# argumentcomputer/lurk-beta

Measured on NVIDIA B200. Metric: Lurk iterations proved/sec (fib rc=100, Nova IVC), higher is better.
Workload: dtype u32x8 (254-bit Montgomery integers)

## Files before the change

lurk-beta_b200/csrc/field.cuh:

```cuda
#pragma once
#include <cstdint>
#include <cstring>

#if defined(__CUDACC__)
#define LURK_HD __host__ __device__ __forceinline__
#define LURK_D __device__ __forceinline__
#else
#define LURK_HD inline
#define LURK_D inline
#endif

#include "field_consts.cuh"

namespace lurk {

namespace cc {
#if defined(__CUDA_ARCH__)
LURK_D uint32_t add_cc(uint32_t a, uint32_t b) { uint32_t r; asm volatile("add.cc.u32 %0, %1, %2;" : "=r"(r) : "r"(a), "r"(b)); return r; }
LURK_D uint32_t addc_cc(uint32_t a, uint32_t b) { uint32_t r; asm volatile("addc.cc.u32 %0, %1, %2;" : "=r"(r) : "r"(a), "r"(b)); return r; }
LURK_D uint32_t addc(uint32_t a, uint32_t b) { uint32_t r; asm volatile("addc.u32 %0, %1, %2;" : "=r"(r) : "r"(a), "r"(b)); return r; }
LURK_D uint32_t sub_cc(uint32_t a, uint32_t b) { uint32_t r; asm volatile("sub.cc.u32 %0, %1, %2;" : "=r"(r) : "r"(a), "r"(b)); return r; }
LURK_D uint32_t subc_cc(uint32_t a, uint32_t b) { uint32_t r; asm volatile("subc.cc.u32 %0, %1, %2;" : "=r"(r) : "r"(a), "r"(b)); return r; }
LURK_D uint32_t subc(uint32_t a, uint32_t b) { uint32_t r; asm volatile("subc.u32 %0, %1, %2;" : "=r"(r) : "r"(a), "r"(b)); return r; }
LURK_D uint32_t mul_lo(uint32_t a, uint32_t b) { uint32_t r; asm volatile("mul.lo.u32 %0, %1, %2;" : "=r"(r) : "r"(a), "r"(b)); return r; }
LURK_D uint32_t mul_hi(uint32_t a, uint32_t b) { uint32_t r; asm volatile("mul.hi.u32 %0, %1, %2;" : "=r"(r) : "r"(a), "r"(b)); return r; }
LURK_D uint32_t mad_lo_cc(uint32_t a, uint32_t b, uint32_t c) { uint32_t r; asm volatile("mad.lo.cc.u32 %0, %1, %2, %3;" : "=r"(r) : "r"(a), "r"(b), "r"(c)); return r; }
LURK_D uint32_t madc_lo_cc(uint32_t a, uint32_t b, uint32_t c) { uint32_t r; asm volatile("madc.lo.cc.u32 %0, %1, %2, %3;" : "=r"(r) : "r"(a), "r"(b), "r"(c)); return r; }
LURK_D uint32_t mad_hi_cc(uint32_t a, uint32_t b, uint32_t c) { uint32_t r; asm volatile("mad.hi.cc.u32 %0, %1, %2, %3;" : "=r"(r) : "r"(a), "r"(b), "r"(c)); return r; }
LURK_D uint32_t madc_hi_cc(uint32_t a, uint32_t b, uint32_t c) { uint32_t r; asm volatile("madc.hi.cc.u32 %0, %1, %2, %3;" : "=r"(r) : "r"(a), "r"(b), "r"(c)); return r; }
LURK_D uint32_t madc_hi(uint32_t a, uint32_t b, uint32_t c) { uint32_t r; asm volatile("madc.hi.u32 %0, %1, %2, %3;" : "=r"(r) : "r"(a), "r"(b), "r"(c)); return r; }
#else
inline uint32_t &cf() { static thread_local uint32_t f = 0; return f; }
inline uint32_t add_cc(uint32_t a, uint32_t b) { uint64_t s = (uint64_t)a + b; cf() = (uint32_t)(s >> 32); return (uint32_t)s; }
inline uint32_t addc_cc(uint32_t a, uint32_t b) { uint64_t s = (uint64_t)a + b + cf(); cf() = (uint32_t)(s >> 32); return (uint32_t)s; }
inline uint32_t addc(uint32_t a, uint32_t b) { return a + b + cf(); }
inline uint32_t sub_cc(uint32_t a, uint32_t b) { uint64_t d = (uint64_t)a - b; cf() = (uint32_t)(d >> 63); return (uint32_t)d; }
inline uint32_t subc_cc(uint32_t a, uint32_t b) { uint64_t d = (uint64_t)a - b - cf(); cf() = (uint32_t)(d >> 63); return (uint32_t)d; }
inline uint32_t subc(uint32_t a, uint32_t b) { return a - b - cf(); }
inline uint32_t mul_lo(uint32_t a, uint32_t b) { return a * b; }
inline uint32_t mul_hi(uint32_t a, uint32_t b) { return (uint32_t)(((uint64_t)a * b) >> 32); }
inline uint32_t mad_lo_cc(uint32_t a, uint32_t b, uint32_t c) { uint64_t s = (uint64_t)(a * b) + c; cf() = (uint32_t)(s >> 32); return (uint32_t)s; }
inline uint32_t madc_lo_cc(uint32_t a, uint32_t b, uint32_t c) { uint64_t s = (uint64_t)(a * b) + c + cf(); cf() = (uint32_t)(s >> 32); return (uint32_t)s; }
inline uint32_t mad_hi_cc(uint32_t a, uint32_t b, uint32_t c) { uint64_t s = (((uint64_t)a * b) >> 32) + c; cf() = (uint32_t)(s >> 32); return (uint32_t)s; }
inline uint32_t madc_hi_cc(uint32_t a, uint32_t b, uint32_t c) { uint64_t s = (((uint64_t)a * b) >> 32) + c + cf(); cf() = (uint32_t)(s >> 32); return (uint32_t)s; }
inline uint32_t madc_hi(uint32_t a, uint32_t b, uint32_t c) { return (uint32_t)(((uint64_t)a * b) >> 32) + c + cf(); }
#endif
}

template <class P>
struct alignas(16) Fe {
    uint32_t v[8];
    using Params = P;

    LURK_HD static Fe zero() { Fe r; for (int i = 0; i < 8; i++) r.v[i] = 0; return r; }
    LURK_HD static Fe one() { Fe r; for (int i = 0; i < 8; i++) r.v[i] = P::ONE(i); return r; }
    LURK_HD static Fe rr() { Fe r; for (int i = 0; i < 8; i++) r.v[i] = P::RR(i); return r; }
    LURK_HD static Fe modulus_raw() { Fe r; for (int i = 0; i < 8; i++) r.v[i] = P::MOD(i); return r; }

    LURK_HD bool is_zero() const { uint32_t o = 0; for (int i = 0; i < 8; i++) o |= v[i]; return o == 0; }
    LURK_HD bool operator==(const Fe &b) const { uint32_t o = 0; for (int i = 0; i < 8; i++) o |= v[i] ^ b.v[i]; return o == 0; }
    LURK_HD bool operator!=(const Fe &b) const { return !(*this == b); }

    LURK_HD void final_sub() {
        uint32_t t[8];
        t[0] = cc::sub_cc(v[0], P::MOD(0));
#pragma unroll
        for (int i = 1; i < 8; i++) t[i] = cc::subc_cc(v[i], P::MOD(i));
        uint32_t borrow = cc::subc(0, 0);
#pragma unroll
        for (int i = 0; i < 8; i++) v[i] = borrow ? v[i] : t[i];
    }
    LURK_HD bool is_reduced() const {
        uint32_t t = cc::sub_cc(v[0], P::MOD(0));
#pragma unroll
        for (int i = 1; i < 8; i++) t = cc::subc_cc(v[i], P::MOD(i));
        (void)t;
        return cc::subc(0, 0) != 0;
    }

    LURK_HD friend Fe operator+(const Fe &a, const Fe &b) {
        Fe r;
        r.v[0] = cc::add_cc(a.v[0], b.v[0]);
#pragma unroll
        for (int i = 1; i < 7; i++) r.v[i] = cc::addc_cc(a.v[i], b.v[i]);
        r.v[7] = cc::addc(a.v[7], b.v[7]);
        r.final_sub();
        return r;
    }
    LURK_HD friend Fe operator-(const Fe &a, const Fe &b) {
        Fe r;
        r.v[0] = cc::sub_cc(a.v[0], b.v[0]);
#pragma unroll
        for (int i = 1; i < 8; i++) r.v[i] = cc::subc_cc(a.v[i], b.v[i]);
        uint32_t borrow = cc::subc(0, 0);
        r.v[0] = cc::add_cc(r.v[0], P::MOD(0) & borrow);
#pragma unroll
        for (int i = 1; i < 7; i++) r.v[i] = cc::addc_cc(r.v[i], P::MOD(i) & borrow);
        r.v[7] = cc::addc(r.v[7], P::MOD(7) & borrow);
        return r;
    }
    LURK_HD Fe neg() const { return zero() - *this; }
    LURK_HD Fe dbl() const { return *this + *this; }

    LURK_HD static void mul_n(uint32_t *acc, const uint32_t *a, uint32_t bi) {
#pragma unroll
        for (int j = 0; j < 8; j += 2) { acc[j] = cc::mul_lo(a[j], bi); acc[j + 1] = cc::mul_hi(a[j], bi); }
    }
    LURK_HD static void cmad_n(uint32_t *acc, const uint32_t *a, uint32_t bi) {
        acc[0] = cc::mad_lo_cc(a[0], bi, acc[0]);
        acc[1] = cc::madc_hi_cc(a[0], bi, acc[1]);
#pragma unroll
        for (int j = 2; j < 8; j += 2) { acc[j] = cc::madc_lo_cc(a[j], bi, acc[j]); acc[j + 1] = cc::madc_hi_cc(a[j], bi, acc[j + 1]); }
    }
    template <int OFF>
    LURK_HD static void cmad_mod(uint32_t *acc, uint32_t mi) {
        acc[0] = cc::mad_lo_cc(P::MOD(OFF), mi, acc[0]);
        acc[1] = cc::madc_hi_cc(P::MOD(OFF), mi, acc[1]);
#pragma unroll
        for (int j = 2; j < 8; j += 2) { acc[j] = cc::madc_lo_cc(P::MOD(OFF + j), mi, acc[j]); acc[j + 1] = cc::madc_hi_cc(P::MOD(OFF + j), mi, acc[j + 1]); }
    }
    LURK_HD static void madc_n_rshift(uint32_t *odd, const uint32_t *a, uint32_t bi) {
#pragma unroll
        for (int j = 0; j < 6; j += 2) { odd[j] = cc::madc_lo_cc(a[j], bi, odd[j + 2]); odd[j + 1] = cc::madc_hi_cc(a[j], bi, odd[j + 3]); }
        odd[6] = cc::madc_lo_cc(a[6], bi, 0);
        odd[7] = cc::madc_hi(a[6], bi, 0);
    }
    template <bool FIRST>
    LURK_HD static void mad_row_redc(uint32_t *even, uint32_t *odd, const uint32_t *a, uint32_t bi) {
        if (FIRST) {
            mul_n(odd, a + 1, bi);
            mul_n(even, a, bi);
        } else {
            even[0] = cc::add_cc(even[0], odd[1]);
            madc_n_rshift(odd, a + 1, bi);
            cmad_n(even, a, bi);
            odd[7] = cc::addc(odd[7], 0);
        }
        uint32_t mi = even[0] * P::M0;
        cmad_mod<1>(odd, mi);
        cmad_mod<0>(even, mi);
        odd[7] = cc::addc(odd[7], 0);
    }

    LURK_HD friend Fe operator*(const Fe &a, const Fe &b) {
#if !defined(__CUDA_ARCH__) && !defined(LURK_HOST_EMULATE_CC)
        return host_mul(a, b);
#else
        uint32_t even[8], odd[8];
        mad_row_redc<true>(even, odd, a.v, b.v[0]);
        mad_row_redc<false>(odd, even, a.v, b.v[1]);
#pragma unroll
        for (int i = 2; i < 8; i += 2) {
            mad_row_redc<false>(even, odd, a.v, b.v[i]);
            mad_row_redc<false>(odd, even, a.v, b.v[i + 1]);
        }
        Fe r;
        r.v[0] = cc::add_cc(even[0], odd[1]);
#pragma unroll
        for (int i = 1; i < 7; i++) r.v[i] = cc::addc_cc(even[i], odd[i + 1]);
        r.v[7] = cc::addc(even[7], 0);
        r.final_sub();
        return r;
#endif
    }
#if !defined(__CUDA_ARCH__)
    static Fe host_mul(const Fe &a, const Fe &b) {
        typedef unsigned __int128 u128;
        uint64_t A[4], B[4], M[4], t[6] = {0, 0, 0, 0, 0, 0};
        for (int i = 0; i < 4; i++) {
            A[i] = (uint64_t)a.v[2 * i] | ((uint64_t)a.v[2 * i + 1] << 32);
            B[i] = (uint64_t)b.v[2 * i] | ((uint64_t)b.v[2 * i + 1] << 32);
            M[i] = (uint64_t)P::MOD(2 * i) | ((uint64_t)P::MOD(2 * i + 1) << 32);
        }
        uint64_t inv = 1;
        for (int i = 0; i < 6; i++) inv *= 2 - M[0] * inv;
        inv = 0 - inv;
        for (int i = 0; i < 4; i++) {
            uint64_t c = 0;
            for (int j = 0; j < 4; j++) { u128 s = (u128)A[j] * B[i] + t[j] + c; t[j] = (uint64_t)s; c = (uint64_t)(s >> 64); }
            u128 s = (u128)t[4] + c; t[4] = (uint64_t)s; t[5] = (uint64_t)(s >> 64);
            uint64_t m = t[0] * inv;
            s = (u128)m * M[0] + t[0]; c = (uint64_t)(s >> 64);
            for (int j = 1; j < 4; j++) { s = (u128)m * M[j] + t[j] + c; t[j - 1] = (uint64_t)s; c = (uint64_t)(s >> 64); }
            s = (u128)t[4] + c; t[3] = (uint64_t)s; t[4] = t[5] + (uint64_t)(s >> 64);
        }
        bool ge = t[4] != 0;
        if (!ge) {
            ge = true;
            for (int i = 3; i >= 0; i--) { if (t[i] > M[i]) break; if (t[i] < M[i]) { ge = false; break; } }
        }
        if (ge) { uint64_t br = 0; for (int i = 0; i < 4; i++) { u128 d = (u128)t[i] - M[i] - br; t[i] = (uint64_t)d; br = (uint64_t)(d >> 64) & 1; } }
        Fe r;
        for (int i = 0; i < 4; i++) { r.v[2 * i] = (uint32_t)t[i]; r.v[2 * i + 1] = (uint32_t)(t[i] >> 32); }
        return r;
    }
#endif
    LURK_HD Fe sqr() const { return *this * *this; }
    LURK_HD Fe pow5() const { Fe x2 = sqr(); Fe x4 = x2.sqr(); return x4 * *this; }

    LURK_HD Fe &operator+=(const Fe &b) { *this = *this + b; return *this; }
    LURK_HD Fe &operator-=(const Fe &b) { *this = *this - b; return *this; }
    LURK_HD Fe &operator*=(const Fe &b) { *this = *this * b; return *this; }

    LURK_HD static Fe from_canonical(const Fe &raw) { return raw * rr(); }
    LURK_HD Fe to_canonical() const {
        Fe o = zero();
        o.v[0] = 1;
        return *this * o;
    }
    LURK_HD static Fe from_u64(uint64_t x) {
        Fe r = zero();
        r.v[0] = (uint32_t)x;
        r.v[1] = (uint32_t)(x >> 32);
        return from_canonical(r);
    }

    LURK_HD Fe pow_raw(const uint32_t e[8]) const {
        Fe acc = one(), base = *this;
        for (int i = 0; i < 256; i++) {
            if ((e[i >> 5] >> (i & 31)) & 1) acc = acc * base;
            base = base.sqr();
        }
        return acc;
    }
    LURK_HD Fe inv_vartime() const {
        if (is_zero()) return zero();
        uint32_t u[8], w[8];
        Fe x1 = zero(), x2 = zero();
        x1.v[0] = 1;
#pragma unroll
        for (int i = 0; i < 8; i++) { u[i] = v[i]; w[i] = P::MOD(i); }
        auto is_one = [](const uint32_t *a) { uint32_t o = a[0] ^ 1u; for (int i = 1; i < 8; i++) o |= a[i]; return o == 0; };
        auto shr1 = [](uint32_t *a) { for (int i = 0; i < 7; i++) a[i] = (a[i] >> 1) | (a[i + 1] << 31); a[7] >>= 1; };
        auto halve = [&](Fe &x) {
            if (x.v[0] & 1u) {
                x.v[0] = cc::add_cc(x.v[0], P::MOD(0));
                for (int i = 1; i < 7; i++) x.v[i] = cc::addc_cc(x.v[i], P::MOD(i));
                x.v[7] = cc::addc(x.v[7], P::MOD(7));
            }
            shr1(x.v);
        };
        auto sub_raw = [](uint32_t *a, const uint32_t *b) {
            a[0] = cc::sub_cc(a[0], b[0]);
            for (int i = 1; i < 8; i++) a[i] = cc::subc_cc(a[i], b[i]);
            return cc::subc(0, 0);
        };
        auto geq = [](const uint32_t *a, const uint32_t *b) {
            for (int i = 7; i >= 0; i--) { if (a[i] > b[i]) return true; if (a[i] < b[i]) return false; }
            return true;
        };
        while (!is_one(u) && !is_one(w)) {
            while (!(u[0] & 1u)) { shr1(u); halve(x1); }
            while (!(w[0] & 1u)) { shr1(w); halve(x2); }
            if (geq(u, w)) { sub_raw(u, w); x1 = x1 - x2; }
            else { sub_raw(w, u); x2 = x2 - x1; }
        }
        const Fe r3 = rr() * rr();
        return (is_one(u) ? x1 : x2) * r3;
    }
    LURK_HD Fe inv() const {
        uint32_t e[8];
        e[0] = cc::sub_cc(P::MOD(0), 2);
#pragma unroll
        for (int i = 1; i < 8; i++) e[i] = cc::subc_cc(P::MOD(i), 0);
        return pow_raw(e);
    }
};

template <class P, int ROUNDS>
LURK_HD Fe<P> redc17(uint32_t *t) {
    uint32_t r[9];
#pragma unroll
    for (int k = 0; k < 9; k++) r[k] = 0;
#pragma unroll
    for (int i = 0; i < 8; i++) {
        uint32_t mi = t[i] * P::M0;
        Fe<P>::template cmad_mod<0>(t + i, mi);
        r[i] = cc::addc(r[i], 0);
        Fe<P>::template cmad_mod<1>(t + i + 1, mi);
        r[i + 1] = cc::addc(r[i + 1], 0);
    }
    t[8] = cc::add_cc(t[8], r[0]);
#pragma unroll
    for (int k = 1; k < 8; k++) t[8 + k] = cc::addc_cc(t[8 + k], r[k]);
    t[16] = cc::addc(t[16], r[8]);
#pragma unroll
    for (int round = 0; round < ROUNDS; round++) {
        uint32_t d[9];
        d[0] = cc::sub_cc(t[8], P::MOD(0));
#pragma unroll
        for (int k = 1; k < 8; k++) d[k] = cc::subc_cc(t[8 + k], P::MOD(k));
        d[8] = cc::subc_cc(t[16], 0);
        uint32_t borrow = cc::subc(0, 0);
#pragma unroll
        for (int k = 0; k < 9; k++) t[8 + k] = borrow ? t[8 + k] : d[k];
    }
    Fe<P> out;
#pragma unroll
    for (int k = 0; k < 8; k++) out.v[k] = t[8 + k];
    return out;
}

template <class P>
struct WideAcc {
    uint32_t e[17];
    uint32_t o[16];
    uint32_t ce[5];
    uint32_t co[4];

    LURK_HD void clear() {
#pragma unroll
        for (int i = 0; i < 17; i++) e[i] = 0;
#pragma unroll
        for (int i = 0; i < 16; i++) o[i] = 0;
#pragma unroll
        for (int i = 0; i < 5; i++) ce[i] = 0;
#pragma unroll
        for (int i = 0; i < 4; i++) co[i] = 0;
    }

    template <int I>
    LURK_HD void row(const uint32_t *a, uint32_t bi) {
        if (I % 2 == 0) {
            Fe<P>::cmad_n(e + I, a, bi);
            ce[I / 2] = cc::addc(ce[I / 2], 0);
            Fe<P>::cmad_n(o + I, a + 1, bi);
            co[I / 2] = cc::addc(co[I / 2], 0);
        } else {
            Fe<P>::cmad_n(e + I + 1, a + 1, bi);
            ce[(I + 1) / 2] = cc::addc(ce[(I + 1) / 2], 0);
            Fe<P>::cmad_n(o + I - 1, a, bi);
            co[(I - 1) / 2] = cc::addc(co[(I - 1) / 2], 0);
        }
    }
    LURK_HD void mul_acc(const Fe<P> &a, const Fe<P> &b) {
        row<0>(a.v, b.v[0]); row<1>(a.v, b.v[1]); row<2>(a.v, b.v[2]); row<3>(a.v, b.v[3]);
        row<4>(a.v, b.v[4]); row<5>(a.v, b.v[5]); row<6>(a.v, b.v[6]); row<7>(a.v, b.v[7]);
    }

    template <int ROUNDS = 3>
    LURK_HD Fe<P> reduce() {
        e[8] = cc::add_cc(e[8], ce[0]);   e[9] = cc::addc_cc(e[9], 0);
        e[10] = cc::addc_cc(e[10], ce[1]); e[11] = cc::addc_cc(e[11], 0);
        e[12] = cc::addc_cc(e[12], ce[2]); e[13] = cc::addc_cc(e[13], 0);
        e[14] = cc::addc_cc(e[14], ce[3]); e[15] = cc::addc_cc(e[15], 0);
        e[16] = cc::addc(e[16], ce[4]);
        o[8] = cc::add_cc(o[8], co[0]);   o[9] = cc::addc_cc(o[9], 0);
        o[10] = cc::addc_cc(o[10], co[1]); o[11] = cc::addc_cc(o[11], 0);
        o[12] = cc::addc_cc(o[12], co[2]); o[13] = cc::addc_cc(o[13], 0);
        o[14] = cc::addc_cc(o[14], co[3]); o[15] = cc::addc(o[15], 0);
        uint32_t t[17];
        t[0] = e[0];
        t[1] = cc::add_cc(e[1], o[0]);
#pragma unroll
        for (int k = 2; k < 16; k++) t[k] = cc::addc_cc(e[k], o[k - 1]);
        t[16] = cc::addc(e[16], o[15]);
        return redc17<P, ROUNDS>(t);
    }
};

template <class F>
LURK_D F load_fe(const void *p) {
#if defined(__CUDA_ARCH__)
    const uint4 *q = reinterpret_cast<const uint4 *>(p);
    uint4 lo = q[0], hi = q[1];
    F r;
    r.v[0] = lo.x; r.v[1] = lo.y; r.v[2] = lo.z; r.v[3] = lo.w;
    r.v[4] = hi.x; r.v[5] = hi.y; r.v[6] = hi.z; r.v[7] = hi.w;
    return r;
#else
    F r; memcpy(r.v, p, 32); return r;
#endif
}
template <class F>
LURK_D void store_fe(void *p, const F &x) {
#if defined(__CUDA_ARCH__)
    uint4 *q = reinterpret_cast<uint4 *>(p);
    q[0] = make_uint4(x.v[0], x.v[1], x.v[2], x.v[3]);
    q[1] = make_uint4(x.v[4], x.v[5], x.v[6], x.v[7]);
#else
    memcpy(p, x.v, 32);
#endif
}

}
```

Before: 27770.

## Replace binary extended GCD inversion with batched safegcd over 30-bit limbs

Replaces the bit-by-bit binary extended Euclid field inverse with a Bernstein–Yang style divstep algorithm. It works on signed 30-bit limbs, runs 30 divsteps per batch on low words, and then applies a 2x2 transition matrix to the full-width values with Montgomery-style division by 2^30. This cuts the number of multi-limb passes and the data-dependent branching per bit. In exchange it adds limb conversion, normalisation, and 64-bit multiply work per batch, and carries correctness risk in the sign, delta and modular-reduction handling.

```diff
diff --git a/lurk-beta_b200/csrc/field.cuh b/lurk-beta_b200/csrc/field.cuh
--- a/lurk-beta_b200/csrc/field.cuh
+++ b/lurk-beta_b200/csrc/field.cuh
@@ -223,40 +223,119 @@
         }
         return acc;
     }
+    static constexpr uint32_t M30 = 0x3fffffffu;
+    LURK_HD static void to_s30(const uint32_t *w, int32_t *o) {
+#pragma unroll
+        for (int k = 0; k < 9; k++) {
+            const int bit = 30 * k, word = bit >> 5, sh = bit & 31;
+            uint32_t lo = w[word] >> sh;
+            if (sh > 2 && word + 1 < 8) lo |= w[word + 1] << (32 - sh);
+            o[k] = (int32_t)(lo & M30);
+        }
+    }
+    LURK_HD static Fe from_s30(const int32_t *o) {
+        Fe r;
+        uint64_t acc = 0;
+        int bits = 0, wi = 0;
+#pragma unroll
+        for (int k = 0; k < 9; k++) {
+            acc |= (uint64_t)(uint32_t)o[k] << bits;
+            bits += 30;
+            if (bits >= 32 && wi < 8) { r.v[wi++] = (uint32_t)acc; acc >>= 32; bits -= 32; }
+        }
+        return r;
+    }
+    LURK_HD static uint32_t ctz32(uint32_t x) {
+#if defined(__CUDA_ARCH__)
+        return (uint32_t)(__ffs((int)x) - 1);
+#else
+        return (uint32_t)__builtin_ctz(x);
+#endif
+    }
+
     LURK_HD Fe inv_vartime() const {
         if (is_zero()) return zero();
-        uint32_t u[8], w[8];
-        Fe x1 = zero(), x2 = zero();
-        x1.v[0] = 1;
-#pragma unroll
-        for (int i = 0; i < 8; i++) { u[i] = v[i]; w[i] = P::MOD(i); }
-        auto is_one = [](const uint32_t *a) { uint32_t o = a[0] ^ 1u; for (int i = 1; i < 8; i++) o |= a[i]; return o == 0; };
-        auto shr1 = [](uint32_t *a) { for (int i = 0; i < 7; i++) a[i] = (a[i] >> 1) | (a[i + 1] << 31); a[7] >>= 1; };
-        auto halve = [&](Fe &x) {
-            if (x.v[0] & 1u) {
-                x.v[0] = cc::add_cc(x.v[0], P::MOD(0));
-                for (int i = 1; i < 7; i++) x.v[i] = cc::addc_cc(x.v[i], P::MOD(i));
-                x.v[7] = cc::addc(x.v[7], P::MOD(7));
+        int32_t f[9], g[9], d[9], e[9], pm[9];
+        {
+            uint32_t w[8];
+#pragma unroll
+            for (int i = 0; i < 8; i++) w[i] = P::MOD(i);
+            to_s30(w, pm);
+        }
+#pragma unroll
+        for (int k = 0; k < 9; k++) { f[k] = pm[k]; d[k] = 0; e[k] = 0; }
+        to_s30(v, g);
+        e[0] = 1;
+        int delta2 = 1;
+        auto normalise = [&pm](int32_t *a) {
+            const int32_t neg = a[8] >> 31;
+            int32_t c = 0;
+#pragma unroll
+            for (int k = 0; k < 8; k++) { c += a[k] + (pm[k] & neg); a[k] = c & (int32_t)M30; c >>= 30; }
+            a[8] += c + (pm[8] & neg);
+            int32_t t[9];
+            c = 0;
+#pragma unroll
+            for (int k = 0; k < 8; k++) { c += a[k] - pm[k]; t[k] = c & (int32_t)M30; c >>= 30; }
+            t[8] = a[8] - pm[8] + c;
+            const int32_t keep = t[8] >> 31;
+#pragma unroll
+            for (int k = 0; k < 9; k++) a[k] = (a[k] & keep) | (t[k] & ~keep);
+        };
+#pragma unroll 1
+        for (int batch = 0; batch < 20; batch++) {
+            uint32_t fl = (uint32_t)f[0], gl = (uint32_t)g[0];
+            uint32_t u = 1, vv = 0, q = 0, r = 1;
+            int left = 30;
+#pragma unroll 1
+            for (;;) {
+                const uint32_t z = ctz32(gl | (1u << left));
+                gl >>= z; u <<= z; vv <<= z;
+                delta2 += 2 * (int)z;
+                left -= (int)z;
+                if (left == 0) break;
+                if (delta2 > 0) {
+                    delta2 = 2 - delta2;
+                    uint32_t t = fl; fl = gl; gl -= t;
+                    t = u; u = q; q -= t;
+                    t = vv; vv = r; r -= t;
+                } else {
+                    delta2 += 2;
+                    gl += fl; q += u; r += vv;
+                }
+                gl >>= 1; u <<= 1; vv <<= 1;
+                if (--left == 0) break;
             }
-            shr1(x.v);
-        };
-        auto sub_raw = [](uint32_t *a, const uint32_t *b) {
-            a[0] = cc::sub_cc(a[0], b[0]);
-            for (int i = 1; i < 8; i++) a[i] = cc::subc_cc(a[i], b[i]);
-            return cc::subc(0, 0);
-        };
-        auto geq = [](const uint32_t *a, const uint32_t *b) {
-            for (int i = 7; i >= 0; i--) { if (a[i] > b[i]) return true; if (a[i] < b[i]) return false; }
-            return true;
-        };
-        while (!is_one(u) && !is_one(w)) {
-            while (!(u[0] & 1u)) { shr1(u); halve(x1); }
-            while (!(w[0] & 1u)) { shr1(w); halve(x2); }
-            if (geq(u, w)) { sub_raw(u, w); x1 = x1 - x2; }
-            else { sub_raw(w, u); x2 = x2 - x1; }
-        }
+            const int64_t U = (int32_t)u, V = (int32_t)vv, Q = (int32_t)q, R = (int32_t)r;
+            int64_t cf = U * f[0] + V * g[0], cg = Q * f[0] + R * g[0];
+            cf >>= 30; cg >>= 30;
+            int64_t cd = U * d[0] + V * e[0], ce = Q * d[0] + R * e[0];
+            const int64_t md = (int64_t)(((uint32_t)cd * P::M0) & M30), me = (int64_t)(((uint32_t)ce * P::M0) & M30);
+            cd += md * pm[0]; ce += me * pm[0];
+            cd >>= 30; ce >>= 30;
+#pragma unroll
+            for (int k = 1; k < 9; k++) {
+                cf += U * f[k] + V * g[k];
+                cg += Q * f[k] + R * g[k];
+                cd += U * d[k] + V * e[k] + md * pm[k];
+                ce += Q * d[k] + R * e[k] + me * pm[k];
+                f[k - 1] = (int32_t)(cf & M30); cf >>= 30;
+                g[k - 1] = (int32_t)(cg & M30); cg >>= 30;
+                d[k - 1] = (int32_t)(cd & M30); cd >>= 30;
+                e[k - 1] = (int32_t)(ce & M30); ce >>= 30;
+            }
+            f[8] = (int32_t)cf; g[8] = (int32_t)cg; d[8] = (int32_t)cd; e[8] = (int32_t)ce;
+            normalise(d);
+            normalise(e);
+            int32_t nz = 0;
+#pragma unroll
+            for (int k = 0; k < 9; k++) nz |= g[k];
+            if (nz == 0) break;
+        }
+        Fe x = from_s30(d);
+        if (f[8] < 0) x = x.neg();
         const Fe r3 = rr() * rr();
-        return (is_one(u) ? x1 : x2) * r3;
+        return x * r3;
     }
     LURK_HD Fe inv() const {
         uint32_t e[8];
```

Result: no change. 27790, median of 6 (+0.1%).
